# antas-marcin/weaviate

Measured on AMD Instinct MI355X. Metric: exact 10-NN QPS + achieved HBM GB/s, 1M×128 L2 flat; 1/2/4/8 GPU scaling, higher is better.
Workload: dtype f32

## Files before the change

### weaviate_amd/csrc/wvg_ctx.hip

```cpp

#include <condition_variable>
#include <thread>
#include <functional>
#include <atomic>
#include <mutex>
#include "wvg_host.hpp"

namespace wvg {

static thread_local std::string g_last_error;

void set_error(const std::string &msg) { g_last_error = msg; }

int fail(int code, const std::string &msg)
{
    g_last_error = msg;
    return code;
}

int StreamSlot::device_scratch(size_t bytes, void **out)
{
    if (bytes > dscratch_bytes) {
        if (dscratch) (void)hipFree(dscratch);
        dscratch = nullptr;
// ... 489 lines not shown
        old = t.screen_pilot_gemm;
        t.screen_pilot_gemm = value;
    } else if (key == 24) {
        old = t.single_path;
        t.single_path = value;
    } else if (key == 25) {
        old = t.stream_variant;
        t.stream_variant = value;
    } else if (key == 26) {
        old = t.screen_pilot_screen;
        t.screen_pilot_screen = value;
    } else if (key == 27) {
        old = t.k1_mq;
        t.k1_mq = value;
    } else if (key == 28 && value > 0) {
        old = t.gather_div;
        t.gather_div = value;
    } else if (key == 29) {
        old = t.screen_warm;
        t.screen_warm = value;
    } else if (key == 30) {
        old = t.screen_warm2;
        t.screen_warm2 = value;
    } else if (key == 31) {
        old = t.filter_zc;
        t.filter_zc = value;
    } else if (key == 32) {
        old = t.screen_pilot_gemm_i8;
        t.screen_pilot_gemm_i8 = value;
    } else if (key == 33) {
        old = t.screen_round;
        t.screen_round = value;
    } else if (key == 34) {
        old = t.qshare;
        t.qshare = value;
    } else if (key == 35 && value >= 0) {
        old = t.qshare_mergers;
        t.qshare_mergers = value;
    } else if (key == 36) {
        old = t.multi_bq_bound;
        t.multi_bq_bound = value;
    } else if (key == 37 && value >= 0) {
        old = t.qshare_seed;
        t.qshare_seed = value;
    } else if (key == 38 && value >= 0) {
        old = t.qshare_seed_tpw;
        t.qshare_seed_tpw = value;
    } else if (key == 39) {
        old = t.qshare_combine;
        t.qshare_combine = value;
    } else if (key == 40) {
        old = t.qshare_screen;
        t.qshare_screen = value;
    }
    return old;
}
#endif

int wvg_measure_hbm_read(wvg_ctx *ctx, uint64_t bytes, uint32_t reps, double *out_gbps)
{
    if (!ctx || !out_gbps) return fail(WVG_ERR_INVALID, "null argument");
    *out_gbps = 0.0;
    bytes = bytes / 4096 * 4096;
    if (bytes == 0 || reps == 0) return fail(WVG_ERR_INVALID, "bytes and reps must be > 0");
    WVG_HIP(hipSetDevice(ctx->device));
    void *buf = nullptr;
    if (hipMalloc(&buf, bytes + 256) != hipSuccess) return fail(WVG_ERR_NOMEM, "probe buffer hipMalloc");
    SlotGuard g(ctx);
    hipEvent_t a = nullptr, b = nullptr;
    auto done = [&](int rc) {
        if (g.slot) (void)hipStreamSynchronize(g.slot->stream);
        if (a) (void)hipEventDestroy(a);
        if (b) (void)hipEventDestroy(b);
        (void)hipFree(buf);
        return rc;
    };
    int rc = ctx->acquire(&g.slot);
    if (rc) return done(rc);
    const hipStream_t s = g.slot->stream;
    float *sink = (float *)((char *)buf + bytes);
    if (hipMemsetAsync(buf, 0, bytes + 256, s) != hipSuccess || hipEventCreate(&a) != hipSuccess ||
        hipEventCreate(&b) != hipSuccess)
        return done(fail(WVG_ERR_DEVICE, "probe setup"));
    double best = 0.0;
    for (int blocks : {1024, 2048, 4096, 8192, -256, -512, -1024, -2048}) {
        for (int w = 0; w < 2; w++)
            if (launch_hbm_read(buf, bytes, blocks, sink, s) != hipSuccess) return done(fail(WVG_ERR_DEVICE, "probe"));
        (void)hipEventRecord(a, s);
        for (uint32_t r = 0; r < reps; r++)
            if (launch_hbm_read(buf, bytes, blocks, sink, s) != hipSuccess) return done(fail(WVG_ERR_DEVICE, "probe"));
        (void)hipEventRecord(b, s);
        float ms = 0.f;
        if (hipEventSynchronize(b) != hipSuccess || hipEventElapsedTime(&ms, a, b) != hipSuccess || ms <= 0.f)
            return done(fail(WVG_ERR_DEVICE, "probe timing"));
        best = std::max(best, (double)bytes * reps / (ms * 1e-3) / 1e9);
    }
    *out_gbps = best;
    return done(WVG_OK);
}

int wvg_profile_start(wvg_ctx *ctx)
{
    if (!ctx) return fail(WVG_ERR_INVALID, "null ctx");
    std::lock_guard<std::mutex> g(ctx->prof_mu);
    ctx->prof_used = 0;
    ctx->profiling.store(true);
// ... 24 lines not shown
```

### weaviate_amd/csrc/wvg_internal.hpp

```cpp
#pragma once

#include <hip/hip_runtime.h>
#include <hip/hip_ext.h>

#include <atomic>
#include <chrono>
#include <condition_variable>
#include <deque>
#include <mutex>
#include <shared_mutex>
#include <string>
#include <vector>

#include "../../include/wvgpu.h"
#include "wvg_common.hpp"

namespace wvg {

void set_error(const std::string &msg);
int fail(int code, const std::string &msg);

#define WVG_HIP(expr)                                                                   \
    do {                                                                                \
        hipError_t _e = (expr);                                                         \
// ... 203 lines not shown
inline int pq_cosched_groups(uint32_t nq, int num_cus)
{
    const int g = num_cus / (int)(nq ? nq : 1) / 8;
    return 8 * (g > 0 ? g : 1);
}
hipError_t launch_scan_f32(const ScanArgs &a, uint64_t *partials, int groups, hipStream_t s);
constexpr uint32_t WVG_STATUS_MERGE_TIMEOUT = 1u;
constexpr uint32_t WVG_RECORDS_TIMEOUT = 0xFFFFFFFFu;
constexpr uint32_t STREAM_QIN_FLOATS = 256;
constexpr int SCAN_WAVES = 4;
struct StreamJob {
    uint64_t *partials;
    uint32_t *arrivals;
    uint32_t arrival_base;
    uint32_t *status;
    uint64_t wait_limit;
    uint32_t groups;
    uint64_t *ids;
    float *dists;
    uint32_t *counts;
    uint4 *records;
    uint32_t tag;
    uint32_t legacy_poll;
    uint32_t *ready;
    uint32_t ready_tag;
    uint32_t row_split;
    alignas(16) float qin[STREAM_QIN_FLOATS];
};
hipError_t launch_scan_f32_stream(const ScanArgs &a, const StreamJob &j, hipStream_t s);
struct QShareArgs {
    const void *data;
    const uint64_t *valid;
    const float *queries;
    uint64_t *partials;
    uint32_t *ready;
    uint32_t *status;
    uint64_t *ids;
    float *dists;
    uint32_t *counts;
    uint64_t id_base, tile_begin, tile_end;
    uint64_t wait_limit;
    uint32_t dim, qpitch, nq, k, groups;
    uint32_t reverse;
    uint32_t plain, cache_tail256;
    int metric;
    uint64_t *seeds;
    uint32_t seed_tiles;
    uint32_t seq_combine;
    uint32_t screen;
    uint16_t *qbf;
    float4 *qconst;
    uint64_t *screen_count;
};
struct QShareFilt {
    const uint64_t *allow;
    uint64_t stride;
    uint64_t t0;
};
bool qshare_supported(int metric, uint32_t dim, int order512);
bool qshare_screened(int metric, uint32_t dim, uint32_t k, uint32_t seed_tiles);
uint32_t qshare_queries_per_pass(uint32_t dim, uint32_t k);
uint32_t qshare_groups(uint64_t ntiles, int num_cus);
uint32_t qshare_seed_tiles(uint32_t dim, uint64_t ntiles, uint32_t groups);
hipError_t launch_qshare_seed(const QShareArgs &a, hipStream_t s, const QShareFilt *f = nullptr);
hipError_t launch_scan_f32_qshare(const QShareArgs &a, uint32_t mergers, hipStream_t s, const QShareFilt *f = nullptr);
struct GroupQuery {
    const void *data;
    const uint64_t *valid;
    uint64_t id_base;
    uint64_t tile_begin, tile_end;
    uint64_t allow_off;
    uint64_t allow_words;
    uint64_t allow_t0;
    uint32_t list0, nlists;
    uint32_t filtered, pad;
};
static_assert(sizeof(GroupQuery) == 80, "descriptor layout shared by host and device");
struct GroupItem {
    uint32_t query, range;
    uint32_t t0, t1;
};
struct GroupArgs {
    const GroupQuery *desc;
    const GroupItem *items;
    const float *queries;
    const uint64_t *allow;
    uint64_t *partials;
    uint32_t qpitch, k, dim, nchunks;
    int metric, order512;
};
hipError_t launch_scan_f32_group(const GroupArgs &a, uint32_t nitems, hipStream_t s);
hipError_t launch_merge_group(const GroupQuery *desc, const uint64_t *partials, uint32_t nq, uint32_t k, uint64_t *ids,
                              float *dists, uint32_t *counts, hipStream_t s);
uint32_t group_item_tiles(uint64_t total_tiles, int num_cus);
hipError_t launch_fill_empty(uint64_t *ids, float *dists, uint32_t *counts, uint32_t nq, uint32_t k, hipStream_t s);
hipError_t launch_scan_bq(const ScanArgs &a, uint64_t *partials, int groups, hipStream_t s);
constexpr int BQ_SCAN_WAVES = 4;
constexpr size_t BQ_EMIT_LDS_MAX = 128u << 10;
hipError_t launch_scan_bq_emit(const ScanArgs &a, uint64_t *partials, int groups, bool lds, hipStream_t s);
hipError_t launch_emit_prefix(const uint64_t *partials, uint32_t nq, uint32_t groups, uint32_t k, float *thr,
                              hipStream_t s, uint32_t max_dist = 0);
hipError_t launch_emit_filter(uint64_t *emit, const uint32_t *emit_cnt, uint32_t emit_cap, const float *thr,
                              uint32_t nq, uint32_t groups, uint32_t waves_per_group, uint32_t *fcnt, uint32_t *oflow,
                              hipStream_t s, const float *bound = nullptr);
hipError_t launch_emit_gather(const uint64_t *emit, const uint32_t *fcnt, uint32_t emit_cap, uint32_t nq,
                              uint32_t waves, uint64_t *out, uint32_t out_cap, uint32_t *totals, hipStream_t s);
bool slab_hist_fits(uint32_t nbins);
hipError_t launch_slab_hist(const uint64_t *partials, uint32_t nq, uint32_t groups, uint32_t k, uint32_t nbins,
                            uint32_t *hist, hipStream_t s);
hipError_t launch_slab_bound(const uint32_t *hists, uint32_t nq, uint32_t nbins, uint32_t R, uint32_t s0, uint32_t ns,
                             float *X, hipStream_t s);
hipError_t launch_scan_pq(const ScanArgs &a, uint64_t *partials, int groups, hipStream_t s);
hipError_t launch_scan_f32_qlist(const ScanArgs &a, uint64_t *partials, int groups, const uint32_t *qlist,
                                 const uint32_t *nlist, uint32_t slots, hipStream_t s);
hipError_t launch_merge_lists_qlist(const uint64_t *partials, uint32_t nq, uint32_t nlists, uint32_t list_len,
                                    uint32_t k, uint64_t id_base, uint64_t *ids, float *dists, uint32_t *counts,
                                    const uint32_t *qlist, const uint32_t *nlist, hipStream_t s);
// ... 40 lines not shown
    int metric = 0;
    const float *data = nullptr;
    uint32_t nchunks = 0;
    const ScanArgs *pilot = nullptr;
    uint64_t *pilot_part = nullptr;
    uint32_t pilot_groups = 1;
    uint32_t pilot_part_lists = 0;
    uint64_t *pilot_ids = nullptr;
    float *pilot_dists = nullptr;
    uint32_t *pilot_counts = nullptr;
};
hipError_t launch_screen(const ScreenLaunch &L, hipStream_t s);
bool gemm_supported(uint32_t dim, int metric);
uint32_t gemm_row_ranges(uint32_t nq, uint64_t ntiles, int num_cus, uint32_t dim, uint32_t k);
hipError_t launch_gemm_topk(const ScanArgs &a, uint32_t nrr, uint64_t *partials, uint32_t *prog, uint32_t *gbound,
                            int num_cus, hipStream_t s);
struct Tuning {
    int scan_variant = 0;
    int groups_per_cu = 0;
    int gemm_pf = 0;
    int gemm_kernel = 0;
    int gemm_lockstep = 0;
    int gemm_skew = 0;
    int pipeline_mode = 1;
    int pq_variant = 0;
    int merge_wait_us = 0;
    int serpentine = 1;
    int k1_loads = 0;
    int gemm_range_tiles = 0;
    int gemm_pairing = 0;
    int gemm_prio = 0;
    int pq_cosched = 1;
    int bq_cos_gpc = 2;
    int k1_tail = 0;
    int pq_encode_min3 = 1;
    int screen_pilot = 16;
    int screen_pilot_gemm = 512;
    int screen_round = 1;
    int screen_pilot_gemm_i8 = 256;
    int screen_variant = 0;
    int stream_variant = 1;
    int single_path = 0;
    int screen_split = 1;
    int screen_seed = 3;
    int screen_range_blocks = 0;
    int gather_div = 4;
    int screen_warm = 32;
    int filter_zc = 1;
    int screen_warm2 = 0;
    int k1_mq = 4;
    int screen_pilot_screen = 0;
    int qshare = 0;
    int qshare_mergers = 0;
    int qshare_seed = 32;
    int qshare_seed_tpw = 124;
    int qshare_combine = 1;
    int qshare_screen = 1;
    int multi_bq_bound = 1;
    int screen_diag = 0;
};
#ifdef WVG_TOOLS
Tuning &tuning();
#else
const Tuning &tuning();
#endif
struct LaunchEvents {
    hipEvent_t start = nullptr, stop = nullptr;
};
LaunchEvents &armed_events();
template <typename... KArgs, typename... Args>
inline void launch_timed(void (*kernel)(KArgs...), dim3 grid, dim3 block, uint32_t lds, hipStream_t s, Args... args)
{
    LaunchEvents &e = armed_events();
    if (e.start) {
        hipExtLaunchKernelGGL(kernel, grid, block, lds, s, e.start, e.stop, 0u, args...);
        e = LaunchEvents{};
    } else {
        hipLaunchKernelGGL(kernel, grid, block, lds, s, args...);
    }
}
constexpr size_t WVG_LDS_BYTES = 160 * 1024;
template <auto Kern>
inline bool fits_lds(size_t dynamic)
{
    static const size_t fixed = [] {
        hipFuncAttributes fa{};
        if (hipFuncGetAttributes(&fa, reinterpret_cast<const void *>(Kern)) != hipSuccess) {
            (void)hipGetLastError();
            return WVG_LDS_BYTES + 1;
        }
        return (size_t)fa.sharedSizeBytes;
    }();
    return fixed + dynamic <= WVG_LDS_BYTES;
}
hipError_t launch_merge_lists(const uint64_t *partials, uint32_t nq, uint32_t nlists, uint32_t list_len, uint32_t k,
                              uint64_t id_base, uint64_t *ids, float *dists, uint32_t *counts, hipStream_t s);
hipError_t launch_merge_keys(const uint64_t *partials, uint32_t nq, uint32_t n_per_query, uint32_t k,
                             uint64_t id_base, uint64_t *ids, float *dists, uint32_t *counts,
                             hipStream_t s);
hipError_t launch_merge_pairs(const float *dists, const uint64_t *ids, uint64_t ids_stride, uint64_t d_stride,
                              uint32_t nq, uint32_t nlists, uint32_t k_in, uint32_t k, uint64_t *out_ids,
                              float *out_dists, uint32_t *out_counts, hipStream_t s);

hipError_t launch_f32_store(const float *rows, const uint64_t *slots, uint64_t n, uint32_t dim,
                            uint32_t nchunks, int normalize, float *tiled, hipStream_t s);
hipError_t launch_f32_synth(uint64_t seed, int dist, uint64_t row0, uint64_t n, uint64_t slot0,
                            uint32_t dim, uint32_t nchunks, int normalize, float *tiled,
// ... 84 lines not shown
```

### weaviate_amd/csrc/wvg_qshare.hip

```cpp
#include <algorithm>

#include "wvg_internal.hpp"
#include "wvg_rowdist.hpp"
#include "wvg_stream.hpp"
#include "wvg_topk.hpp"

namespace wvg {

typedef __attribute__((address_space(4))) const f4v cf4;
typedef __attribute__((address_space(4))) const uint64_t cu64;

typedef float f2v __attribute__((ext_vector_type(2)));

template <int METRIC>
__device__ __forceinline__ void chunk_update2(f2v (&acc)[4][4], int cc, f4v q, float4 x)
{
    const int r = cc >> 1, p = (cc & 1) * 2;
    const f2v qlo = {q.x, q.y}, qhi = {q.z, q.w}, xlo = {x.x, x.y}, xhi = {x.z, x.w};
    if constexpr (METRIC == WVG_M_L2) {
        const f2v dl = qlo - xlo, dh = qhi - xhi;
        acc[r][p] = __builtin_elementwise_fma(dl, dl, acc[r][p]);
        acc[r][p + 1] = __builtin_elementwise_fma(dh, dh, acc[r][p + 1]);
    } else {
        acc[r][p] = __builtin_elementwise_fma(qlo, xlo, acc[r][p]);
// ... 16 lines not shown

__device__ __forceinline__ void ld_granule(f4v (&q)[4], cf4 *p)
{
#pragma unroll
    for (int i = 0; i < 4; i++) q[i] = p[i];
}

constexpr int qshare_qp(int d, int e, bool whole)
{
    return whole ? (e == 1 ? 16 : (e == 2 ? 8 : 4)) : ((d == 0 || d > 128) && e == 4 ? 2 : 4);
}

__device__ __forceinline__ uint64_t seed_bound(cu64 *seed)
{
    const uint64_t s = *seed;
    return s + (s != WVG_KEY_NONE ? 1ull : 0ull);
}

typedef float floatx4 __attribute__((ext_vector_type(4)));
typedef __bf16 bf16x2 __attribute__((ext_vector_type(2)));
typedef short shortx4 __attribute__((ext_vector_type(4)));
constexpr int QS_D = 128;
constexpr double QS_C = 0x1p-7 + 0x1p-15 + QS_D * 0x1p-21;
constexpr float QS_G = 0x1p-15f;
constexpr int QS_QROW = QS_D * 2 / 16 + 1;
constexpr int QS_FROW = QS_D / 4 + 1;

__device__ __forceinline__ shortx4 bf16_of(float4 x)
{
    const bf16x2 lo = __builtin_convertvector(f2v{x.x, x.y}, bf16x2), hi = __builtin_convertvector(f2v{x.z, x.w}, bf16x2);
    return __builtin_bit_cast(shortx4, make_uint2(__builtin_bit_cast(uint32_t, lo), __builtin_bit_cast(uint32_t, hi)));
}

__device__ __forceinline__ void screen_query_side(const QShareArgs &a, uint32_t q, cf4 *qj, int lane)
{
    const int c = lane & (QS_D / 4 - 1);
    const f4v v = qj[c];
    double ss = lane < QS_D / 4
                    ? (double)v.x * (double)v.x + (double)v.y * (double)v.y + (double)v.z * (double)v.z + (double)v.w * (double)v.w
                    : 0.0;
#pragma unroll
    for (int off = 32; off > 0; off >>= 1) ss += __shfl_xor(ss, off);
    if (lane < QS_D / 4)
        reinterpret_cast<shortx4 *>(a.qbf)[(size_t)q * (QS_D / 4) + c] = bf16_of(make_float4(v.x, v.y, v.z, v.w));
    if (lane == 0) {
        const double nq = __builtin_sqrt(ss) * (1.0 + 1e-6);
        const double k1 = (2.0 * QS_C * nq + 0x1p-60) * (1.0 + 0x1p-20);
        const double k2 = (double)QS_G * ss + 0x1p-60 * nq + 0x1p-100;
        a.qconst[q] = make_float4((float)ss, (float)k1, (float)k2, (float)(ss - k2));
    }
}

constexpr int SEED_WAVES = 16;

__device__ __forceinline__ uint64_t allow_word(cu64 *aq, uint64_t stride, uint64_t t0, uint64_t t)
{
    const uint64_t w = t - t0;
    return w < stride ? aq[w] : 0ull;
}

template <int METRIC, int D, int E, bool FILT>
__device__ __forceinline__ void qshare_seed_body(const QShareArgs &a, const QShareFilt &f, uint32_t bdim, uint32_t gdim)
{
    static_assert(D % 32 == 0 && D > 0 && !is_abs_or_neq<METRIC>, "shared rows: fixed D, the AVX2 chains");
    constexpr int NC = D / 4;
    const uint64_t nready = (uint64_t)a.nq * a.groups;
    for (uint64_t i = (uint64_t)blockIdx.x * bdim + threadIdx.x; i < nready; i += (uint64_t)gdim * bdim)
        a.ready[i] = 0u;
    const uint32_t q = blockIdx.x;
    const int lane = threadIdx.x & 63, wave = wave_id();
    cf4 *qj = (cf4 *)a.queries + (size_t)q * (a.qpitch / 4);
    if constexpr (METRIC == WVG_M_L2 && D == QS_D) {
        if (a.screen) {
#ifdef WVG_TOOLS
            if (threadIdx.x == 0 && q == 0) a.screen_count[0] = a.screen_count[1] = 0ull;
#endif
            if (wave == SEED_WAVES - 1) screen_query_side(a, q, qj, lane);
        }
    }
    const uint64_t ntiles = a.tile_end - a.tile_begin;
    const uint64_t ns = a.seed_tiles < ntiles ? a.seed_tiles : ntiles;
    if (ns == 0) {
        if (threadIdx.x == 0) a.seeds[q] = WVG_KEY_NONE;
        return;
    }
    const float4 *data = reinterpret_cast<const float4 *>(a.data);
    cu64 *valid = (cu64 *)a.valid;
    cu64 *aq = FILT ? (cu64 *)f.allow + (size_t)q * f.stride : nullptr;
    WaveTopK<E> tk;
    tk.init((int)a.k);
    for (uint64_t t = a.tile_begin + (uint64_t)wave; t < a.tile_begin + ns; t += SEED_WAVES) {
        uint64_t m = valid[t];
        if constexpr (FILT) m &= allow_word(aq, f.stride, f.t0, t);
        if (m == 0ull) continue;
        const float4 *rp = data + (size_t)t * NC * 64 + lane;
        f2v acc[4][4];
#pragma unroll
        for (int r = 0; r < 4; r++)
#pragma unroll
            for (int p = 0; p < 4; p++) acc[r][p] = f2v{0.0f, 0.0f};
#pragma unroll 2
        for (int b = 0; b < D / 32; b++) {
            float4 xs[8];
#pragma unroll
            for (int cc = 0; cc < 8; cc++) xs[cc] = rp[(size_t)(b * 8 + cc) * 64];
#pragma unroll
            for (int cc = 0; cc < 8; cc++) chunk_update2<METRIC>(acc, cc, qj[b * 8 + cc], xs[cc]);
        }
        tk.offer(lane_key(m, wrap_metric(a.metric, avx256_reduce2(acc)), t, lane));
    }
    const uint64_t kth = group_combine_kth<E, SEED_WAVES>(tk);
    if (threadIdx.x == 0) a.seeds[q] = kth;
}

template <int METRIC, int D, int E>
__global__ __launch_bounds__(SEED_WAVES * 64) void qshare_seed_kernel(QShareArgs a)
{
    qshare_seed_body<METRIC, D, E, false>(a, QShareFilt{}, blockDim.x, gridDim.x);
}

template <int METRIC, int D, int E>
__global__ __launch_bounds__(SEED_WAVES * 64) void qshare_seed_filt_kernel(QShareArgs a, QShareFilt f)
{
    qshare_seed_body<METRIC, D, E, true>(a, f, blockDim.x, gridDim.x);
}

__global__ __launch_bounds__(SEED_WAVES * 64) void qshare_open_seed_kernel(QShareArgs a)
{
    const uint64_t nready = (uint64_t)a.nq * a.groups;
    for (uint64_t i = (uint64_t)blockIdx.x * blockDim.x + threadIdx.x; i < nready; i += (uint64_t)gridDim.x * blockDim.x)
        a.ready[i] = 0u;
    if (threadIdx.x == 0) a.seeds[blockIdx.x] = WVG_KEY_NONE;
}

template <int E, int QP, bool FRESH = false>
__device__ __forceinline__ void pass_combine_publish(WaveTopK<E> (&tk)[QP], uint32_t nqp, uint32_t k, uint64_t *partials,
                                                     uint32_t *ready, size_t list0, uint32_t G, bool more)
{
    __shared__ uint64_t psh[QP][SCAN_WAVES][64 * E];
    int lane = threadIdx.x & 63;
    if constexpr (FRESH) asm volatile("" : "+v"(lane));
    const int wave = wave_id();
#pragma unroll
    for (int j = 0; j < QP; j++)
#pragma unroll
        for (int e = 0; e < E; e++) psh[j][wave][e * 64 + lane] = tk[j].l[e];
    __syncthreads();
    for (uint32_t j = (uint32_t)wave; j < nqp; j += SCAN_WAVES) {
        uint64_t l[E];
#pragma unroll
        for (int e = 0; e < E; e++) l[e] = psh[j][0][e * 64 + lane];
#pragma unroll
        for (int w = 1; w < SCAN_WAVES; w++) {
            uint64_t o[E];
#pragma unroll
            for (int e = 0; e < E; e++) o[e] = psh[j][w][e * 64 + lane];
            merge_lists<E>(l, o);
        }
        const size_t li = list0 + (size_t)j * G;
        uint64_t *out = partials + li * k;
#pragma unroll
        for (int e = 0; e < E; e++) {
            const uint32_t i = e * 64 + lane;
            if (i < k) __hip_atomic_store((gu64 *)(out + i), l[e], __ATOMIC_RELAXED, __HIP_MEMORY_SCOPE_AGENT);
        }
        asm volatile("s_waitcnt vmcnt(0)" ::: "memory");
        if (lane == 0) __hip_atomic_store((gu32 *)(ready + li), 1u, __ATOMIC_RELAXED, __HIP_MEMORY_SCOPE_AGENT);
    }
    if (more) __syncthreads();
}

template <int QP, bool FILT>
__device__ __forceinline__ uint32_t screen_tile(const float4 (&xs)[QS_D / 4], const uint4 *qsh, cf4 *kq,
                                                const WaveTopK<1> (&tk)[QP], uint32_t nqp, uint64_t m,
                                                const uint64_t (&mq)[FILT ? QP : 1], int lane)
{
    static_assert(QP == 16, "four query groups of four");
// ... 326 lines not shown
template <int METRIC, int E>
__global__ __launch_bounds__(SCAN_WAVES * 64) __attribute__((amdgpu_waves_per_eu(2, 2))) void scan_f32_qshare_dyn_filt_kernel(
    QShareArgs a, QShareFilt f)
{
    qshare_scan_body<METRIC, 0, E, false, false, true>(a, f);
}

__global__ __launch_bounds__(SCAN_WAVES * 64) __attribute__((amdgpu_waves_per_eu(2, 2))) void scan_f32_qshare_screen_kernel(
    QShareArgs a)
{
    qshare_scan_body<WVG_M_L2, QS_D, 1, true, true, false>(a, QShareFilt{});
}

__global__ __launch_bounds__(SCAN_WAVES * 64) __attribute__((amdgpu_waves_per_eu(2, 2))) void scan_f32_qshare_screen_filt_kernel(
    QShareArgs a, QShareFilt f)
{
    qshare_scan_body<WVG_M_L2, QS_D, 1, true, true, true>(a, f);
}

bool qshare_supported(int metric, uint32_t dim, int order512)
{
    return (metric == WVG_M_L2 || metric == WVG_M_DOT || metric == WVG_M_COSINE) && dim % 4 == 0 && dim >= 8 &&
           !order512;
}

static int qshare_fixed_dim(uint32_t dim)
{
#ifdef WVG_TOOLS
    if (tuning().qshare == 3) return 0;
#endif
    return dim == 128 || dim == 768 ? (int)dim : 0;
}

static bool qshare_whole(uint32_t dim)
{
#ifdef WVG_TOOLS
    if (tuning().qshare == 2) return false;
#endif
    return qshare_fixed_dim(dim) == 128;
}

uint32_t qshare_queries_per_pass(uint32_t dim, uint32_t k)
{
    const int e = k <= 64 ? 1 : (k <= 128 ? 2 : 4);
    return (uint32_t)qshare_qp(qshare_fixed_dim(dim), e, qshare_whole(dim));
}

uint32_t qshare_groups(uint64_t ntiles, int num_cus)
{
    const uint64_t g = std::min<uint64_t>((uint64_t)num_cus * 2, (ntiles + SCAN_WAVES - 1) / SCAN_WAVES);
    return (uint32_t)std::max<uint64_t>(g, 1);
}

uint32_t qshare_seed_tiles(uint32_t dim, uint64_t ntiles, uint32_t groups)
{
    const Tuning &t = tuning();
    if (t.qshare_seed <= 0 || dim != 128 || groups == 0) return 0;
    if (ntiles / ((uint64_t)groups * SCAN_WAVES) > (uint64_t)t.qshare_seed_tpw) return 0;
    return (uint32_t)std::min<uint64_t>((uint64_t)t.qshare_seed, ntiles);
}

bool qshare_screened(int metric, uint32_t dim, uint32_t k, uint32_t seed_tiles)
{
    return tuning().qshare_screen != 0 && metric == WVG_M_L2 && dim == (uint32_t)QS_D && k <= 64 && seed_tiles > 0 &&
           qshare_whole(dim);
}

template <int METRIC, int E>
static hipError_t launch_seed_e(const QShareArgs &a, hipStream_t s, const QShareFilt *f)
{
    dim3 grid(a.nq), block(SEED_WAVES * 64);
    if (a.dim != 128 && a.dim != 768) {
        if (a.seed_tiles || a.screen) return hipErrorInvalidValue;
        hipLaunchKernelGGL(qshare_open_seed_kernel, grid, block, 0, s, a);
        return hipGetLastError();
    }
    if (f) {
        if (a.dim == 128)
            hipLaunchKernelGGL((qshare_seed_filt_kernel<METRIC, 128, E>), grid, block, 0, s, a, *f);
        else
            hipLaunchKernelGGL((qshare_seed_filt_kernel<METRIC, 768, E>), grid, block, 0, s, a, *f);
    } else if (a.dim == 128) {
        hipLaunchKernelGGL((qshare_seed_kernel<METRIC, 128, E>), grid, block, 0, s, a);
    } else {
        hipLaunchKernelGGL((qshare_seed_kernel<METRIC, 768, E>), grid, block, 0, s, a);
    }
    return hipGetLastError();
}

hipError_t launch_qshare_seed(const QShareArgs &a, hipStream_t s, const QShareFilt *f)
{
    if (!qshare_supported(a.metric, a.dim, 0) || a.nq == 0) return hipErrorInvalidValue;
    auto go = [&](auto M) -> hipError_t {
        constexpr int MM = decltype(M)::value;
        if (a.k <= 64) return launch_seed_e<MM, 1>(a, s, f);
        if (a.k <= 128) return launch_seed_e<MM, 2>(a, s, f);
        return launch_seed_e<MM, 4>(a, s, f);
    };
    return a.metric == WVG_M_L2 ? go(MetricTag<WVG_M_L2>{}) : go(MetricTag<WVG_M_DOT>{});
}

template <int METRIC, int E>
static hipError_t launch_qshare_e(const QShareArgs &a, uint32_t mergers, hipStream_t s, const QShareFilt *f)
{
    dim3 grid(a.groups + mergers), block(SCAN_WAVES * 64);
    if (a.screen) {
        if (METRIC != WVG_M_L2 || E != 1 || a.dim != QS_D || !a.qbf || !a.qconst) return hipErrorInvalidValue;
        if (f)
            launch_timed(scan_f32_qshare_screen_filt_kernel, grid, block, 0, s, a, *f);
        else
            launch_timed(scan_f32_qshare_screen_kernel, grid, block, 0, s, a);
        return hipGetLastError();
    }
    if (qshare_fixed_dim(a.dim) == 0) {
        if (f)
            launch_timed((scan_f32_qshare_dyn_filt_kernel<METRIC, E>), grid, block, 0, s, a, *f);
        else
            launch_timed((scan_f32_qshare_dyn_kernel<METRIC, E>), grid, block, 0, s, a);
        return hipGetLastError();
    }
    if (f) {
        if (a.dim == 128)
            launch_timed((scan_f32_qshare_filt_kernel<METRIC, 128, E, true>), grid, block, 0, s, a, *f);
        else if (a.dim == 768)
            launch_timed((scan_f32_qshare_filt_kernel<METRIC, 768, E, false>), grid, block, 0, s, a, *f);
        else
            return hipErrorInvalidValue;
        return hipGetLastError();
    }
    if (a.dim == 128) {
#ifdef WVG_TOOLS
        if (!qshare_whole(a.dim)) {
            launch_timed((scan_f32_qshare_kernel<METRIC, 128, E, false>), grid, block, 0, s, a);
            return hipGetLastError();
        }
#endif
        launch_timed((scan_f32_qshare_kernel<METRIC, 128, E, true>), grid, block, 0, s, a);
    } else if (a.dim == 768) {
        launch_timed((scan_f32_qshare_kernel<METRIC, 768, E, false>), grid, block, 0, s, a);
    } else {
        return hipErrorInvalidValue;
    }
    return hipGetLastError();
}

hipError_t launch_scan_f32_qshare(const QShareArgs &a, uint32_t mergers, hipStream_t s, const QShareFilt *f)
{
    if (!qshare_supported(a.metric, a.dim, 0) || mergers == 0) return hipErrorInvalidValue;
    auto go = [&](auto M) -> hipError_t {
        constexpr int MM = decltype(M)::value;
// ... 9 lines not shown
```

### weaviate_amd/csrc/wvg_search.hip

```cpp

#include <atomic>
#include <chrono>

#include "wvg_host.hpp"

namespace wvg {

static void normalize_host(const float *v, uint32_t n, float *out)
{
    float norm = 0.0f;
    for (uint32_t i = 0; i < n; i++) {
        float p = v[i] * v[i];
        norm = norm + p;
    }
    if (norm == 0.0f) {
        for (uint32_t i = 0; i < n; i++) out[i] = 0.0f;
        return;
    }
    norm = (float)std::sqrt((double)norm);
    for (uint32_t i = 0; i < n; i++) out[i] = v[i] / norm;
}

static void normalize_host_rows(const float *v, uint32_t nq, uint32_t d, float *out, uint32_t pitch)
{
// ... 1029 lines not shown
    a.dim = d;
    a.nchunks = bq->nchunks;
    a.metric = bq->metric;
    a.queries = b + o_qb;
    a.qpitch = qpb;
    a.nq = nq;
    a.k = R;
    a.cosched = p.cosched;
    a.reverse = next_direction(bq, 1);
    uint64_t *part = (uint64_t *)(b + o_part);
    WVG_HIP(launch_scan_bq(a, part, p.groups, s));
    uint64_t *cand_ids = (uint64_t *)(b + o_cand);
    WVG_HIP(launch_merge_lists(part, nq, (uint32_t)p.groups, R, R, 0, cand_ids, (float *)(b + o_resc), nullptr, s));
    WVG_HIP(launch_rescore_keys(f32->metric, (const float *)(b + o_qf), qpf, (const float *)f32->d_data, d,
                                f32->nchunks, cand_ids, nq, R, R, (uint64_t *)(b + o_resc), s, f32->ctx->order512));
    WVG_HIP(launch_merge_keys((uint64_t *)(b + o_resc), nq, R, k, f32->id_base, (uint64_t *)(b + o_ids),
                              (float *)(b + o_d), (uint32_t *)(b + o_cnt), s));
    if (out_ids) WVG_HIP(hipMemcpyAsync(out_ids, b + o_ids, (size_t)nq * k * 8, hipMemcpyDeviceToHost, s));
    if (out_dists) WVG_HIP(hipMemcpyAsync(out_dists, b + o_d, (size_t)nq * k * 4, hipMemcpyDeviceToHost, s));
    if (out_counts) WVG_HIP(hipMemcpyAsync(out_counts, b + o_cnt, (size_t)nq * 4, hipMemcpyDeviceToHost, s));
    WVG_HIP(hipStreamSynchronize(s));
    return WVG_OK;
}

int wvg_search_bq_candidates(wvg_corpus *bq, const float *queries, uint32_t nq, uint32_t rescore_limit,
                             const uint64_t *allow_bits, uint64_t allow_words, uint64_t *out_ids, float *out_dists,
                             uint32_t *out_counts)
{
    int rc = check_corpus(bq);
    if (rc) return rc;
    if (bq->kind != WVG_KIND_BQ) return fail(WVG_ERR_INVALID, "need a BQ corpus");
    if (nq > 0 && !queries) return fail(WVG_ERR_INVALID, "null queries");
    const uint32_t R = rescore_limit;
    if (!bq->ctx->opt.heap_replay) {
        rc = wvg_search(bq, queries, nq, R, allow_bits, allow_words, out_ids, out_dists, out_counts);
        if (rc) return rc;
        for (uint32_t q = 0; q < nq; q++) {
            const uint32_t c = out_counts ? out_counts[q] : R;
            if (out_ids) std::reverse(out_ids + (size_t)q * R, out_ids + (size_t)q * R + c);
            if (out_dists) std::reverse(out_dists + (size_t)q * R, out_dists + (size_t)q * R + c);
        }
        return WVG_OK;
    }
    std::shared_lock<std::shared_mutex> lk(bq->rw);
    SearchPlan p = plan_search(bq, nq, std::min(R, MAX_K), allow_bits, allow_words);
    if (p.empty || R == 0) {
        write_empty(nq, R, out_ids, out_dists, out_counts);
        return WVG_OK;
    }
    return bq_rescore_replay(bq, nullptr, queries, nq, R, R, p, out_ids, out_dists, out_counts);
}

static const size_t WS_STATUS_BYTES = 256;

struct StreamLayout {
    size_t partials = 0, arrivals = 0, ready = 0, total = 0;
};
static StreamLayout stream_layout(const SearchPlan &p1, uint32_t nq, uint32_t k)
{
    StreamLayout l;
    l.partials = WS_STATUS_BYTES;
    l.arrivals = l.partials + align_up((size_t)nq * p1.groups * k * 8, 256);
    l.ready = l.arrivals + align_up((size_t)nq * 4, 256);
    l.total = l.ready + align_up((size_t)nq * p1.groups * 4, 256);
    return l;
}

struct QShareLayout {
    size_t partials = 0, ready = 0, seeds = 0, qbf = 0, qconst = 0, count = 0, total = 0;
    uint32_t groups = 0;
};
static QShareLayout qshare_layout(const wvg_corpus *c, const SearchPlan &p1, uint32_t nq, uint32_t k)
{
    QShareLayout l;
    l.groups = qshare_groups(p1.te - p1.tb, c->ctx->num_cus);
    l.partials = WS_STATUS_BYTES;
    l.ready = l.partials + align_up((size_t)nq * l.groups * k * 8, 256);
    l.seeds = l.ready + align_up((size_t)nq * l.groups * 4, 256);
    l.qbf = l.seeds + align_up((size_t)nq * 8, 256);
    l.qconst = l.qbf + (c->dim == 128 ? align_up((size_t)nq * 128 * 2, 256) : 0);
    l.count = l.qconst + (c->dim == 128 ? align_up((size_t)nq * 16, 256) : 0);
    l.total = l.count + 256;
    return l;
}

static bool qshare_route(const wvg_corpus *c, uint32_t nq)
{
    if (tuning().qshare < 0) return false;
    return nq >= 2 && c->kind == WVG_KIND_F32 && c->ctx->opt.cache_reuse &&
           qshare_supported(c->metric, c->dim, c->ctx->order512);
}

static wvg_stream_plan stream_plan(const wvg_corpus *c, const SearchPlan &p1, uint32_t nq, uint32_t k, uint32_t *seed_tiles)
{
    wvg_stream_plan sp{0u, 1u, p1.empty ? 0u : nq, 0u, 0u};
    *seed_tiles = 0;
    if (p1.empty || tuning().pipeline_mode != 1 || !qshare_route(c, nq)) return sp;
    sp.shared_rows = 1;
    sp.queries_per_pass = qshare_queries_per_pass(c->dim, k);
    sp.passes = (nq + sp.queries_per_pass - 1) / sp.queries_per_pass;
    *seed_tiles = qshare_seed_tiles(c->dim, p1.te - p1.tb, qshare_groups(p1.te - p1.tb, c->ctx->num_cus));
    sp.seeded = *seed_tiles > 0;
    sp.screened = c->ctx->qshare_screen && qshare_screened(c->metric, c->dim, k, *seed_tiles);
    return sp;
}

int wvg_search_device_pipelined_plan(wvg_corpus *c, uint32_t nq, uint32_t k, wvg_stream_plan *out)
{
    if (!c || !out) return fail(WVG_ERR_INVALID, "null corpus / plan");
    if (k > MAX_K) return fail(WVG_ERR_UNSUPPORTED, "k above 256 is not supported by the fused top-k");
    if (c->kind != WVG_KIND_F32) return fail(WVG_ERR_UNSUPPORTED, "pipelined search supports F32 corpora");
    if (c->dim % 4 != 0) return fail(WVG_ERR_UNSUPPORTED, "device search needs dim % 4 == 0");
    *out = wvg_stream_plan{0u, 1u, 0u, 0u, 0u};
    if (nq == 0 || k == 0) return WVG_OK;
    std::shared_lock<std::shared_mutex> lk(c->rw);
    uint32_t seed_tiles;
    *out = stream_plan(c, plan_search(c, 1, k, nullptr, 0), nq, k, &seed_tiles);
    return WVG_OK;
}

size_t wvg_search_workspace_size(wvg_corpus *c, uint32_t nq, uint32_t k)
{
    if (!c) return 0;
    const uint32_t kk = std::max<uint32_t>(k, 1);
    SearchPlan p = plan_search(c, nq, k, nullptr, 0);
    const size_t dev = WS_STATUS_BYTES + align_up(p.workspace_bytes(nq, kk), 256) + device_query_bytes(c, nq);
    if (c->kind != WVG_KIND_F32) return dev;
    SearchPlan p1 = plan_search(c, 1, k, nullptr, 0);
    const size_t chain = 2 * align_up(p1.workspace_bytes(1, kk), 256);
    const size_t stream = stream_layout(p1, nq, kk).total;
    const size_t shared = qshare_layout(c, p1, nq, kk).total;
    return std::max({dev, WS_STATUS_BYTES + chain, stream, shared});
}

#ifdef WVG_TOOLS
// ... 47 lines not shown
{
    if (!c) return fail(WVG_ERR_INVALID, "null corpus");
    if (k > MAX_K) return fail(WVG_ERR_UNSUPPORTED, "k above 256 is not supported by the fused top-k");
    if (c->kind != WVG_KIND_F32) return fail(WVG_ERR_UNSUPPORTED, "pipelined search supports F32 corpora");
    if (c->dim % 4 != 0) return fail(WVG_ERR_UNSUPPORTED, "device search needs dim % 4 == 0");
    if (nq == 0 || k == 0) return WVG_OK;
    hipStream_t s = (hipStream_t)stream;
    std::shared_lock<std::shared_mutex> lk(c->rw);
    SearchPlan p = plan_search(c, 1, k, nullptr, 0);
    if (p.empty || (flt && flt->stride == 0)) {
        WVG_HIP(launch_fill_empty(d_ids, d_dists, d_counts, nq, k, s));
        return WVG_OK;
    }
    uint32_t seed_tiles;
    const wvg_stream_plan sp = stream_plan(c, p, nq, k, &seed_tiles);
    if (sp.shared_rows) {
        const QShareLayout l = qshare_layout(c, p, nq, k);
        if (!d_workspace || workspace_bytes < l.total) return fail(WVG_ERR_INVALID, "workspace too small");
        char *w = (char *)d_workspace;
        QShareArgs a{};
        a.data = c->d_data;
        a.valid = c->d_valid;
        a.queries = d_queries;
        a.partials = (uint64_t *)(w + l.partials);
        a.ready = (uint32_t *)(w + l.ready);
        a.status = (uint32_t *)w;
        a.ids = d_ids;
        a.dists = d_dists;
        a.counts = d_counts;
        a.id_base = c->id_base;
        a.tile_begin = p.tb;
        a.tile_end = p.te;
        const uint32_t wait_us = tuning().merge_wait_us > 0 ? (uint32_t)tuning().merge_wait_us : c->ctx->opt.merge_wait_us;
        a.wait_limit = wait_us > 0 ? (uint64_t)wait_us * 100ull : 400000000ull;
        a.dim = c->dim;
        a.qpitch = c->dim;
        a.nq = nq;
        a.k = k;
        a.groups = l.groups;
        a.reverse = next_direction(c, sp.passes);
        a.plain = plain_loads(c, p.tb, p.te);
        a.cache_tail256 = k1_cache_tail(c, p.tb, p.te);
        a.metric = c->metric;
        const uint32_t mergers = tuning().qshare_mergers > 0 ? (uint32_t)tuning().qshare_mergers : std::min<uint32_t>(nq, 64);
        a.seeds = (uint64_t *)(w + l.seeds);
        a.seed_tiles = seed_tiles;
        a.seq_combine = tuning().qshare_combine == 0;
        a.screen = sp.screened;
        if (a.screen) {
            a.qbf = (uint16_t *)(w + l.qbf);
            a.qconst = (float4 *)(w + l.qconst);
            a.screen_count = (uint64_t *)(w + l.count);
        }
        WVG_HIP(launch_qshare_seed(a, s, flt));
        ProfArm arm(c->ctx);
        if (arm.rc) return arm.rc;
        WVG_HIP(launch_scan_f32_qshare(a, mergers, s, flt));
        return WVG_OK;
    }
    if (flt && nq > 1) {
        const StreamLayout l = stream_layout(p, nq, k);
        if (!d_workspace || workspace_bytes < l.total) return fail(WVG_ERR_INVALID, "workspace too small");
        uint64_t *partials = (uint64_t *)((char *)d_workspace + l.partials);
        ScanArgs a{};
        a.data = c->d_data;
        a.valid = c->d_valid;
        a.allow = flt->allow;
        a.allow_words = flt->stride;
        a.allow_t0 = flt->t0;
        a.allow_qstride = flt->stride;
        a.id_base = c->id_base;
        a.tile_begin = p.tb;
        a.tile_end = p.te;
        a.dim = c->dim;
        a.nchunks = c->nchunks;
        a.metric = c->metric;
        a.queries = d_queries;
        a.qpitch = c->dim;
        a.nq = nq;
        a.k = k;
        a.reverse = next_direction(c, 1);
        a.order512 = c->ctx->order512;
        a.plain = plain_loads(c, p.tb, p.te);
        a.cache_tail256 = k1_cache_tail(c, p.tb, p.te);
        ProfArm arm(c->ctx);
        if (arm.rc) return arm.rc;
        WVG_HIP(launch_scan_f32(a, partials, p.groups, s));
        WVG_HIP(launch_merge_lists(partials, nq, (uint32_t)p.groups, k, k, c->id_base, d_ids, d_dists, d_counts, s));
        return WVG_OK;
    }
    if (tuning().pipeline_mode == 1) {
        const StreamLayout l = stream_layout(p, nq, k);
        if (!d_workspace || workspace_bytes < l.total) return fail(WVG_ERR_INVALID, "workspace too small");
        char *w = (char *)d_workspace;
        StreamJob j{};
        j.partials = (uint64_t *)(w + l.partials);
        j.arrivals = (uint32_t *)(w + l.arrivals);
        j.status = (uint32_t *)w;
        const uint32_t wait_us = tuning().merge_wait_us > 0 ? (uint32_t)tuning().merge_wait_us : c->ctx->opt.merge_wait_us;
        j.wait_limit = wait_us > 0 ? (uint64_t)wait_us * 100ull : 400000000ull;
        j.groups = (uint32_t)p.groups;
        j.ids = d_ids;
        j.dists = d_dists;
        j.counts = d_counts;
        ScanArgs a{};
        a.data = c->d_data;
        a.valid = c->d_valid;
// ... 251 lines not shown
```

Before: 129,900.

## Parallelize qshare seed kernel across tiles with last-block merge of per-tile lists

The seed kernel used to run one 16-wave block per query, with each wave walking seed tiles serially. Now the grid is tiles × query-blocks, one wave per query, and each wave scores a single tile and writes its sorted top-k list to a workspace buffer. The last block to arrive on one of 16 arrival counters merges those lists into the k-th-key seed, with early termination by ballot. The default seed tile count rises to 64, capped by a per-corpus share, which trades more seeding work for tighter thresholds but adds atomic counters, extra workspace and a serial merge tail.

```diff
diff --git a/weaviate_amd/csrc/wvg_ctx.hip b/weaviate_amd/csrc/wvg_ctx.hip
--- a/weaviate_amd/csrc/wvg_ctx.hip
+++ b/weaviate_amd/csrc/wvg_ctx.hip
@@ -565,6 +565,9 @@
     } else if (key == 40) {
         old = t.qshare_screen;
         t.qshare_screen = value;
+    } else if (key == 41 && value >= 1) {
+        old = t.qshare_seed_share;
+        t.qshare_seed_share = value;
     }
     return old;
 }
diff --git a/weaviate_amd/csrc/wvg_internal.hpp b/weaviate_amd/csrc/wvg_internal.hpp
--- a/weaviate_amd/csrc/wvg_internal.hpp
+++ b/weaviate_amd/csrc/wvg_internal.hpp
@@ -279,6 +279,11 @@
     float4 *qconst;
     uint64_t *screen_count;
 };
+constexpr uint32_t PRO_COUNTERS = 16;
+struct QSharePro {
+    uint64_t *lists;
+    uint32_t *arrivals;
+};
 struct QShareFilt {
     const uint64_t *allow;
     uint64_t stride;
@@ -289,7 +294,7 @@
 uint32_t qshare_queries_per_pass(uint32_t dim, uint32_t k);
 uint32_t qshare_groups(uint64_t ntiles, int num_cus);
 uint32_t qshare_seed_tiles(uint32_t dim, uint64_t ntiles, uint32_t groups);
-hipError_t launch_qshare_seed(const QShareArgs &a, hipStream_t s, const QShareFilt *f = nullptr);
+hipError_t launch_qshare_seed(const QShareArgs &a, const QSharePro &pro, hipStream_t s, const QShareFilt *f = nullptr);
 hipError_t launch_scan_f32_qshare(const QShareArgs &a, uint32_t mergers, hipStream_t s, const QShareFilt *f = nullptr);
 struct GroupQuery {
     const void *data;
@@ -436,7 +441,8 @@
     int screen_pilot_screen = 0;
     int qshare = 0;
     int qshare_mergers = 0;
-    int qshare_seed = 32;
+    int qshare_seed = 64;
+    int qshare_seed_share = 64;
     int qshare_seed_tpw = 124;
     int qshare_combine = 1;
     int qshare_screen = 1;
diff --git a/weaviate_amd/csrc/wvg_qshare.hip b/weaviate_amd/csrc/wvg_qshare.hip
--- a/weaviate_amd/csrc/wvg_qshare.hip
+++ b/weaviate_amd/csrc/wvg_qshare.hip
@@ -92,6 +92,8 @@
 }
 
 constexpr int SEED_WAVES = 16;
+constexpr int PRO_WAVES = 8;
+constexpr int PRO_CHUNK = 12;
 
 __device__ __forceinline__ uint64_t allow_word(cu64 *aq, uint64_t stride, uint64_t t0, uint64_t t)
 {
@@ -100,69 +102,131 @@
 }
 
 template <int METRIC, int D, int E, bool FILT>
-__device__ __forceinline__ void qshare_seed_body(const QShareArgs &a, const QShareFilt &f, uint32_t bdim, uint32_t gdim)
+__device__ __forceinline__ void qshare_seed_body(const QShareArgs &a, const QSharePro &pro, const QShareFilt &f,
+                                                 uint32_t bdim, uint32_t gdim)
 {
     static_assert(D % 32 == 0 && D > 0 && !is_abs_or_neq<METRIC>, "shared rows: fixed D, the AVX2 chains");
     constexpr int NC = D / 4;
+    constexpr bool WHOLE = D <= 128;
     const uint64_t nready = (uint64_t)a.nq * a.groups;
     for (uint64_t i = (uint64_t)blockIdx.x * bdim + threadIdx.x; i < nready; i += (uint64_t)gdim * bdim)
         a.ready[i] = 0u;
-    const uint32_t q = blockIdx.x;
     const int lane = threadIdx.x & 63, wave = wave_id();
-    cf4 *qj = (cf4 *)a.queries + (size_t)q * (a.qpitch / 4);
+    const uint32_t T = a.seed_tiles ? a.seed_tiles : 1u;
+    const uint32_t ti = blockIdx.x % T, q = blockIdx.x / T * PRO_WAVES + (uint32_t)wave;
+    const bool hasq = q < a.nq;
+    const uint64_t ntiles = a.tile_end - a.tile_begin;
+    const uint64_t ns = a.seed_tiles < ntiles ? a.seed_tiles : ntiles;
+    const uint64_t t = a.tile_begin + ti;
+    const bool score = hasq && ti < ns;
+    cf4 *qj = (cf4 *)a.queries + (size_t)(hasq ? q : 0u) * (a.qpitch / 4);
+    const float4 *rp = reinterpret_cast<const float4 *>(a.data) + (size_t)t * NC * 64 + lane;
+    float4 xs[WHOLE ? NC : 1];
+    if constexpr (WHOLE) {
+        if (score) {
+#pragma unroll
+            for (int c = 0; c < NC; c++) xs[c] = rp[(size_t)c * 64];
+        }
+    }
     if constexpr (METRIC == WVG_M_L2 && D == QS_D) {
         if (a.screen) {
 #ifdef WVG_TOOLS
-            if (threadIdx.x == 0 && q == 0) a.screen_count[0] = a.screen_count[1] = 0ull;
-#endif
-            if (wave == SEED_WAVES - 1) screen_query_side(a, q, qj, lane);
-        }
-    }
-    const uint64_t ntiles = a.tile_end - a.tile_begin;
-    const uint64_t ns = a.seed_tiles < ntiles ? a.seed_tiles : ntiles;
+            if (threadIdx.x == 0 && blockIdx.x == 0) a.screen_count[0] = a.screen_count[1] = 0ull;
+#endif
+            if (ti == 0 && hasq) screen_query_side(a, q, qj, lane);
+        }
+    }
     if (ns == 0) {
-        if (threadIdx.x == 0) a.seeds[q] = WVG_KEY_NONE;
+        if (hasq && lane == 0) a.seeds[q] = WVG_KEY_NONE;
         return;
     }
-    const float4 *data = reinterpret_cast<const float4 *>(a.data);
-    cu64 *valid = (cu64 *)a.valid;
-    cu64 *aq = FILT ? (cu64 *)f.allow + (size_t)q * f.stride : nullptr;
-    WaveTopK<E> tk;
-    tk.init((int)a.k);
-    for (uint64_t t = a.tile_begin + (uint64_t)wave; t < a.tile_begin + ns; t += SEED_WAVES) {
-        uint64_t m = valid[t];
-        if constexpr (FILT) m &= allow_word(aq, f.stride, f.t0, t);
-        if (m == 0ull) continue;
-        const float4 *rp = data + (size_t)t * NC * 64 + lane;
-        f2v acc[4][4];
-#pragma unroll
-        for (int r = 0; r < 4; r++)
-#pragma unroll
-            for (int p = 0; p < 4; p++) acc[r][p] = f2v{0.0f, 0.0f};
+    uint64_t key = WVG_KEY_NONE;
+    if (score) {
+        uint64_t m = ((cu64 *)a.valid)[t];
+        if constexpr (FILT) m &= allow_word((cu64 *)f.allow + (size_t)q * f.stride, f.stride, f.t0, t);
+        if (m != 0ull) {
+            f2v acc[4][4];
+#pragma unroll
+            for (int r = 0; r < 4; r++)
+#pragma unroll
+                for (int p = 0; p < 4; p++) acc[r][p] = f2v{0.0f, 0.0f};
+            if constexpr (WHOLE) {
+#pragma unroll
+                for (int c = 0; c < NC; c++) chunk_update2<METRIC>(acc, c & 7, qj[c], xs[c]);
+            } else {
 #pragma unroll 2
-        for (int b = 0; b < D / 32; b++) {
-            float4 xs[8];
-#pragma unroll
-            for (int cc = 0; cc < 8; cc++) xs[cc] = rp[(size_t)(b * 8 + cc) * 64];
-#pragma unroll
-            for (int cc = 0; cc < 8; cc++) chunk_update2<METRIC>(acc, cc, qj[b * 8 + cc], xs[cc]);
-        }
-        tk.offer(lane_key(m, wrap_metric(a.metric, avx256_reduce2(acc)), t, lane));
-    }
-    const uint64_t kth = group_combine_kth<E, SEED_WAVES>(tk);
-    if (threadIdx.x == 0) a.seeds[q] = kth;
+                for (int b = 0; b < D / 32; b++) {
+                    float4 xb[8];
+#pragma unroll
+                    for (int cc = 0; cc < 8; cc++) xb[cc] = rp[(size_t)(b * 8 + cc) * 64];
+#pragma unroll
+                    for (int cc = 0; cc < 8; cc++) chunk_update2<METRIC>(acc, cc, qj[b * 8 + cc], xb[cc]);
+                }
+            }
+            key = lane_key(m, wrap_metric(a.metric, avx256_reduce2(acc)), t, lane);
+            sort64(key);
+        }
+    }
+    const uint32_t kk = a.k < 64u ? a.k : 64u;
+    if (hasq && (uint32_t)lane < kk)
+        __hip_atomic_store((gu64 *)(pro.lists + ((size_t)q * T + ti) * kk + lane), key, __ATOMIC_RELAXED,
+                           __HIP_MEMORY_SCOPE_AGENT);
+    asm volatile("s_waitcnt vmcnt(0)" ::: "memory");
+    __shared__ uint32_t last_sh;
+    __shared__ uint64_t stage[PRO_WAVES][PRO_CHUNK][64];
+    __syncthreads();
+    const uint32_t nqb = (a.nq + PRO_WAVES - 1) / PRO_WAVES, qb = blockIdx.x / T, cls = qb % PRO_COUNTERS;
+    gu32 *ctr = (gu32 *)pro.arrivals + cls;
+    if (threadIdx.x == 0) {
+        const uint32_t want = T * ((nqb - cls + PRO_COUNTERS - 1) / PRO_COUNTERS);
+        last_sh = __hip_atomic_fetch_add(ctr, 1u, __ATOMIC_RELAXED, __HIP_MEMORY_SCOPE_AGENT) == want - 1u;
+    }
+    __syncthreads();
+    if (!last_sh) return;
+    if (threadIdx.x == 0) __hip_atomic_store(ctr, 0u, __ATOMIC_RELAXED, __HIP_MEMORY_SCOPE_AGENT);
+    for (uint32_t mq = cls * PRO_WAVES + (uint32_t)wave; mq < a.nq; mq += PRO_COUNTERS * PRO_WAVES) {
+        WaveTopK<E> tk;
+        tk.init((int)a.k);
+        for (uint32_t g0 = 0; g0 < T; g0 += 64) {
+            const uint32_t list = g0 + lane;
+            const bool have = list < T;
+            const gu64 *lp = (const gu64 *)(pro.lists + ((size_t)mq * T + (have ? list : 0u)) * kk);
+            for (uint32_t r0 = 0; r0 < kk; r0 += PRO_CHUNK) {
+                uint64_t c[PRO_CHUNK];
+#pragma unroll
+                for (int i = 0; i < PRO_CHUNK; i++)
+                    c[i] = have && r0 + i < kk ? __hip_atomic_load(lp + r0 + i, __ATOMIC_RELAXED, __HIP_MEMORY_SCOPE_AGENT)
+                                               : WVG_KEY_NONE;
+#pragma unroll
+                for (int i = 0; i < PRO_CHUNK; i++) stage[wave][i][lane] = c[i];
+                const uint32_t n = kk - r0 < (uint32_t)PRO_CHUNK ? kk - r0 : (uint32_t)PRO_CHUNK;
+                bool stop = false;
+#pragma unroll 1
+                for (uint32_t i = 0; i < n; i++) {
+                    const uint64_t key = stage[wave][i][lane];
+                    if (r0 + i > 0 && __ballot(key < tk.tau) == 0ull) {
+                        stop = true;
+                        break;
+                    }
+                    tk.offer(key);
+                }
+                if (stop) break;
+            }
+        }
+        if (lane == 0) a.seeds[mq] = tk.tau;
+    }
 }
 
 template <int METRIC, int D, int E>
-__global__ __launch_bounds__(SEED_WAVES * 64) void qshare_seed_kernel(QShareArgs a)
-{
-    qshare_seed_body<METRIC, D, E, false>(a, QShareFilt{}, blockDim.x, gridDim.x);
+__global__ __launch_bounds__(PRO_WAVES * 64) void qshare_seed_kernel(QShareArgs a, QSharePro pro)
+{
+    qshare_seed_body<METRIC, D, E, false>(a, pro, QShareFilt{}, blockDim.x, gridDim.x);
 }
 
 template <int METRIC, int D, int E>
-__global__ __launch_bounds__(SEED_WAVES * 64) void qshare_seed_filt_kernel(QShareArgs a, QShareFilt f)
-{
-    qshare_seed_body<METRIC, D, E, true>(a, f, blockDim.x, gridDim.x);
+__global__ __launch_bounds__(PRO_WAVES * 64) void qshare_seed_filt_kernel(QShareArgs a, QSharePro pro, QShareFilt f)
+{
+    qshare_seed_body<METRIC, D, E, true>(a, pro, f, blockDim.x, gridDim.x);
 }
 
 __global__ __launch_bounds__(SEED_WAVES * 64) void qshare_open_seed_kernel(QShareArgs a)
@@ -595,12 +659,14 @@
     return (uint32_t)std::max<uint64_t>(g, 1);
 }
 
+constexpr uint64_t QSHARE_SEED_FLOOR = 32;
 uint32_t qshare_seed_tiles(uint32_t dim, uint64_t ntiles, uint32_t groups)
 {
     const Tuning &t = tuning();
     if (t.qshare_seed <= 0 || dim != 128 || groups == 0) return 0;
     if (ntiles / ((uint64_t)groups * SCAN_WAVES) > (uint64_t)t.qshare_seed_tpw) return 0;
-    return (uint32_t)std::min<uint64_t>((uint64_t)t.qshare_seed, ntiles);
+    const uint64_t share = std::max<uint64_t>(QSHARE_SEED_FLOOR, ntiles / (uint64_t)std::max(t.qshare_seed_share, 1));
+    return (uint32_t)std::min({(uint64_t)t.qshare_seed, share, ntiles});
 }
 
 bool qshare_screened(int metric, uint32_t dim, uint32_t k, uint32_t seed_tiles)
@@ -610,35 +676,38 @@
 }
 
 template <int METRIC, int E>
-static hipError_t launch_seed_e(const QShareArgs &a, hipStream_t s, const QShareFilt *f)
-{
-    dim3 grid(a.nq), block(SEED_WAVES * 64);
+static hipError_t launch_seed_e(const QShareArgs &a, const QSharePro &pro, hipStream_t s, const QShareFilt *f)
+{
     if (a.dim != 128 && a.dim != 768) {
         if (a.seed_tiles || a.screen) return hipErrorInvalidValue;
-        hipLaunchKernelGGL(qshare_open_seed_kernel, grid, block, 0, s, a);
+        hipLaunchKernelGGL(qshare_open_seed_kernel, dim3(a.nq), dim3(SEED_WAVES * 64), 0, s, a);
         return hipGetLastError();
     }
+    if (a.seed_tiles && (!pro.lists || !pro.arrivals)) return hipErrorInvalidValue;
+    const uint64_t nwg = (uint64_t)(a.seed_tiles ? a.seed_tiles : 1u) * ((a.nq + PRO_WAVES - 1) / PRO_WAVES);
+    if (nwg > 0x7FFFFFFFull) return hipErrorInvalidValue;
+    dim3 grid((uint32_t)nwg), block(PRO_WAVES * 64);
     if (f) {
         if (a.dim == 128)
-            hipLaunchKernelGGL((qshare_seed_filt_kernel<METRIC, 128, E>), grid, block, 0, s, a, *f);
+            hipLaunchKernelGGL((qshare_seed_filt_kernel<METRIC, 128, E>), grid, block, 0, s, a, pro, *f);
         else
-            hipLaunchKernelGGL((qshare_seed_filt_kernel<METRIC, 768, E>), grid, block, 0, s, a, *f);
+            hipLaunchKernelGGL((qshare_seed_filt_kernel<METRIC, 768, E>), grid, block, 0, s, a, pro, *f);
     } else if (a.dim == 128) {
-        hipLaunchKernelGGL((qshare_seed_kernel<METRIC, 128, E>), grid, block, 0, s, a);
+        hipLaunchKernelGGL((qshare_seed_kernel<METRIC, 128, E>), grid, block, 0, s, a, pro);
     } else {
-        hipLaunchKernelGGL((qshare_seed_kernel<METRIC, 768, E>), grid, block, 0, s, a);
+        hipLaunchKernelGGL((qshare_seed_kernel<METRIC, 768, E>), grid, block, 0, s, a, pro);
     }
     return hipGetLastError();
 }
 
-hipError_t launch_qshare_seed(const QShareArgs &a, hipStream_t s, const QShareFilt *f)
+hipError_t launch_qshare_seed(const QShareArgs &a, const QSharePro &pro, hipStream_t s, const QShareFilt *f)
 {
     if (!qshare_supported(a.metric, a.dim, 0) || a.nq == 0) return hipErrorInvalidValue;
     auto go = [&](auto M) -> hipError_t {
         constexpr int MM = decltype(M)::value;
-        if (a.k <= 64) return launch_seed_e<MM, 1>(a, s, f);
-        if (a.k <= 128) return launch_seed_e<MM, 2>(a, s, f);
-        return launch_seed_e<MM, 4>(a, s, f);
+        if (a.k <= 64) return launch_seed_e<MM, 1>(a, pro, s, f);
+        if (a.k <= 128) return launch_seed_e<MM, 2>(a, pro, s, f);
+        return launch_seed_e<MM, 4>(a, pro, s, f);
     };
     return a.metric == WVG_M_L2 ? go(MetricTag<WVG_M_L2>{}) : go(MetricTag<WVG_M_DOT>{});
 }
diff --git a/weaviate_amd/csrc/wvg_search.hip b/weaviate_amd/csrc/wvg_search.hip
--- a/weaviate_amd/csrc/wvg_search.hip
+++ b/weaviate_amd/csrc/wvg_search.hip
@@ -1105,6 +1105,8 @@
 }
 
 static const size_t WS_STATUS_BYTES = 256;
+static const size_t WS_SEED_ARRIVALS = 128;
+static_assert(WS_SEED_ARRIVALS + PRO_COUNTERS * 4 <= WS_STATUS_BYTES, "the counters lie inside the status block");
 
 struct StreamLayout {
     size_t partials = 0, arrivals = 0, ready = 0, total = 0;
@@ -1120,8 +1122,8 @@
 }
 
 struct QShareLayout {
-    size_t partials = 0, ready = 0, seeds = 0, qbf = 0, qconst = 0, count = 0, total = 0;
-    uint32_t groups = 0;
+    size_t partials = 0, ready = 0, seeds = 0, qbf = 0, qconst = 0, count = 0, lists = 0, total = 0;
+    uint32_t groups = 0, seed_tiles = 0;
 };
 static QShareLayout qshare_layout(const wvg_corpus *c, const SearchPlan &p1, uint32_t nq, uint32_t k)
 {
@@ -1133,7 +1135,9 @@
     l.qbf = l.seeds + align_up((size_t)nq * 8, 256);
     l.qconst = l.qbf + (c->dim == 128 ? align_up((size_t)nq * 128 * 2, 256) : 0);
     l.count = l.qconst + (c->dim == 128 ? align_up((size_t)nq * 16, 256) : 0);
-    l.total = l.count + 256;
+    l.lists = l.count + 256;
+    l.seed_tiles = qshare_seed_tiles(c->dim, p1.te - p1.tb, l.groups);
+    l.total = l.lists + align_up((size_t)nq * l.seed_tiles * std::min<uint32_t>(k, 64) * 8, 256);
     return l;
 }
 
@@ -1287,7 +1291,8 @@
             a.qconst = (float4 *)(w + l.qconst);
             a.screen_count = (uint64_t *)(w + l.count);
         }
-        WVG_HIP(launch_qshare_seed(a, s, flt));
+        const QSharePro pro{(uint64_t *)(w + l.lists), (uint32_t *)(w + WS_SEED_ARRIVALS)};
+        WVG_HIP(launch_qshare_seed(a, pro, s, flt));
         ProfArm arm(c->ctx);
         if (arm.rc) return arm.rc;
         WVG_HIP(launch_scan_f32_qshare(a, mergers, s, flt));
```

Result: faster. 139,900 (median of 6 runs) (+7.7%).
